# NumericalEarth/Breeze.jl

Measured on AMD Instinct MI355X. Metric: grid-cells advanced/sec (tendency+Poisson step), 512^3 anelastic, higher is better.
Workload: dtype f64

## Files before the change

### breeze.jl_amd/csrc/bz_tendency5_kernels.h

```cpp
#pragma once
#include "bz_internal.h"
#include "bz_weno.h"
#include "bz_tendency4_kernels.h"

#ifndef BZ_KO
#define BZ_KO 0
#endif
#ifndef BZ6_ROTATE_DUTY
#define BZ6_ROTATE_DUTY 0
#endif
#ifndef BZ6_UNROLL2
#define BZ6_UNROLL2 0
#endif
#ifndef BZ6_LDS_BARRIER
#define BZ6_LDS_BARRIER 0
#endif
__device__ __forceinline__ void bz6_barrier()
{
#if BZ6_LDS_BARRIER
    __builtin_amdgcn_fence(__ATOMIC_RELEASE, "workgroup", "local");
    __builtin_amdgcn_s_barrier();
    __builtin_amdgcn_fence(__ATOMIC_ACQUIRE, "workgroup", "local");
#else
    __syncthreads();
#endif
}
typedef long long ix_t;
typedef unsigned ix32_t;

struct LevRow5 {
    double rho, rrho;
    double rho_f, rrho_f;
    double Ax, Ay, Vinv_c;
    double pi;
    double Vinv_f, T_r;
    double pad[6];
};
struct Lev5 {
    const LevRow5 *p;
#ifdef __HIPCC__
    __device__ __forceinline__ double at(int k, int f) const { return ((ColPtr::cptr)(const double *)p)[(long long)k * 16 + f]; }
    __device__ __forceinline__ double rho(int k) const { return at(k, 0); }
    __device__ __forceinline__ double rrho(int k) const { return at(k, 1); }
    __device__ __forceinline__ double rho_f(int k) const { return at(k, 2); }
    __device__ __forceinline__ double rrho_f(int k) const { return at(k, 3); }
    __device__ __forceinline__ double Ax(int k) const { return at(k, 4); }
    __device__ __forceinline__ double Ay(int k) const { return at(k, 5); }
    __device__ __forceinline__ double Vinv_c(int k) const { return at(k, 6); }
    __device__ __forceinline__ double pi(int k) const { return at(k, 7); }
    __device__ __forceinline__ double Vinv_f(int k) const { return at(k, 8); }
    __device__ __forceinline__ double T_r(int k) const { return at(k, 9); }
#endif
};
static_assert(sizeof(LevRow5) == 16 * sizeof(double), "LevRow5 is sixteen reals");

#ifndef BZ_LEAN_WAVES
#define BZ_LEAN_WAVES (sizeof(double) == 8 ? 4 : 6)
#endif
#ifndef BZ5_ZERO_SHORTCUT
#define BZ5_ZERO_SHORTCUT 1
#endif
#ifndef BZ5_TOPS_AHEAD
#define BZ5_TOPS_AHEAD 1
#endif
#ifndef BZ6_W_WAVES
#define BZ6_W_WAVES 4
#endif
#ifndef BZ5_EB
#define BZ5_EB 64
#endif
#ifndef BZ5_RAW_LDS
#define BZ5_RAW_LDS 0
#endif
#ifndef BZ5_SCALAR_WAVES
#define BZ5_SCALAR_WAVES (sizeof(double) == 8 ? 4 : 6)
#endif

struct Lean5 {
    const double *ru, *rv, *rw;
    const double *pa, *pb;
    double *out;
    double *oa, *ob;
    double *T;
    ColPtr pi_dry;
    const LevRow5 *lev;
    int mforce;
    double cor_f;
    ColPtr Fu, Fv;
    ColPtr Su, Sv;
    const double *vel, *bT, *bq;
    const int *qstate;
    int xcd;
    int by0, bys;
};

__device__ __forceinline__ void bz_block5(const Lean5 &L, int &bx, int &by, int &bz)
{
    bx = blockIdx.x; by = blockIdx.y; bz = blockIdx.z;
    if (L.xcd) {
        const unsigned gx = gridDim.x, gy = gridDim.y;
        const unsigned W = gx * gy * gridDim.z;
        unsigned w = bx + gx * (by + gy * bz);
        w = (w & 7u) * (W >> 3) + (w >> 3);
        bx = (int)(w % gx);
        by = (int)((w / gx) % gy);
        bz = (int)(w / (gx * gy));
    }
    by = L.by0 + by * L.bys;
    bx = __builtin_amdgcn_readfirstlane(bx);
    by = __builtin_amdgcn_readfirstlane(by);
    bz = __builtin_amdgcn_readfirstlane(bz);
}

__device__ __forceinline__ void st_img5(double *__restrict__ f, long long n, double v, long long ox, long long oy)
{
    f[n] = v;
    if (ox) f[n + ox] = v;
    if (oy) {
        f[n + oy] = v;
        if (ox) f[n + ox + oy] = v;
    }
}


__device__ __forceinline__ double bz_temperature5(const DevGrid &g, double rth, double rq, int k, const ColPtr pi_dry)
{
    const double rho = g.rho[k], rrho = g.rrho[k];
    const double th = bz_cdiv(rth, rho, rrho), q = bz_cdiv(rq, rho, rrho);
    if (pi_dry.p && __all(q == 0.0)) return pi_dry[k] * th;
    const double qd = 1.0 - q;
    const double cpm = qd * g.cpd + q * g.cpv;
    return bz_exner_factor(g, k, q, cpm) * th;
}

__device__ __forceinline__ double bz_temperature5r(const DevGrid &g, double rth, double rq, int k, double rho, double rrho, double pi)
{
    const double th = bz_cdiv(rth, rho, rrho), q = bz_cdiv(rq, rho, rrho);
    if (__all(q == 0.0)) return pi * th;
    const double qd = 1.0 - q;
    const double cpm = qd * g.cpd + q * g.cpv;
    return bz_exner_factor(g, k, q, cpm) * th;
}

template <bool WY> __device__ __forceinline__ int by5_face(const DevGrid &g, int j) { return WY ? bz_buffer_face(j, g.Ny) : 3; }
template <bool WY> __device__ __forceinline__ int by5_center(const DevGrid &g, int j) { return WY ? bz_buffer_center(j, g.Ny) : 3; }
template <bool WY>
__device__ __forceinline__ double bz_up5y(double m3, double m2, double m1, double p0, double p1, double p2, bool left, int B)
{
    if constexpr (WY) return bz_upB(m3, m2, m1, p0, p1, p2, left, B);
    else return bz_up5(m3, m2, m1, p0, p1, p2, left);
}
template <bool WY>
__device__ __forceinline__ double bz_symm4y(double qm2, double qm1, double q0, double qp1, int B)
{
    if constexpr (WY) return (B == 3) ? bz_symm4(qm2, qm1, q0, qp1) : bz_symm2(qm1, q0);
    else return bz_symm4(qm2, qm1, q0, qp1);
}

template <int TY, bool WY, bool DRYQ>
__device__ __forceinline__ void k5_scalar_pair_body(const DevGrid &g, const Lean5 &F, int kchunk, const RKEpilogue &E, double *Tp, double *FYp, int *ZF, double *RAWp)
{
    constexpr bool Q = !DRYQ;
    constexpr int TR = TY + 6, TC = 72;
    constexpr int NHALO = TR * 70 - TY * 64;
    constexpr int NT = 64 * TY;
    constexpr int HPT = (NHALO + NT - 1) / NT;
    double(*T)[2][TR][TC] = (double(*)[2][TR][TC])Tp;
    double(*FY)[2][TY + 1][64] = (double(*)[2][TY + 1][64])FYp;
    double *__restrict__ RAW = RAWp;
    constexpr bool ZS = BZ5_ZERO_SHORTCUT && Q;

    int bx, by, bz;
    bz_block5(F, bx, by, bz);
    const int tx = threadIdx.x, ty = threadIdx.y, t = ty * 64 + tx;
    const int tyu = __builtin_amdgcn_readfirstlane(ty);
    const Lev5 LV{F.lev};
    const int i0 = bx * 64, j0 = by * TY;
    const int i = i0 + tx, j = j0 + ty;
    const int ic = min(i, g.Nx + 2), jc = min(j, g.Ny + 2);
    const int nact = min(64, g.Nx - i0);
    const int ie = i0 + nact, le = nact - 1;
    const int kbeg = bz * kchunk, kend = min(kbeg + kchunk, g.Nz);
    if (kbeg >= kend) return;
    const int Byj = by5_face<WY>(g, j0 + tyu), Byt = by5_face<WY>(g, j0 + TY);
    const unsigned sz = (unsigned)g.Sxy;
    const bool store = (i < g.Nx) && (j < g.Ny);
    const double *__restrict__ ru = F.ru, *__restrict__ rv = F.rv, *__restrict__ rw = F.rw;
    const double *__restrict__ pa = F.pa, *__restrict__ pb = F.pb;
    unsigned n = (unsigned)g.idx(ic, jc, kbeg);

    int hr[HPT], hc[HPT];
    unsigned hn[HPT];
    bool hok[HPT];
#pragma unroll
    for (int q = 0; q < HPT; ++q) {
        const int h = t + q * NT;
        hok[q] = h < NHALO;
        int r, c;
        if (h < 6 * 70) {
            const int rr = h / 70;
            c = h - rr * 70;
            r = (rr < 3) ? rr : TY + rr;
        } else {
            const int hh = h - 6 * 70;
            const int rr = hh / 6, cc = hh - rr * 6;
            r = 3 + rr;
            c = (cc < 3) ? cc : 64 + cc;
        }
        if (!hok[q]) { r = 0; c = 0; }
        hr[q] = r; hc[q] = c;
        const int gi = min(i0 - 3 + c, g.Nx + 2), gj = min(j0 - 3 + r, g.Ny + 2);
        hn[q] = (unsigned)g.idx(gi, gj, kbeg);
    }
    const unsigned ntop0 = (unsigned)g.idx(ic, min(j0 + TY, g.Ny), kbeg);

    double a[6], b[6];
    double araw[3] = {0.0, 0.0, 0.0};
#pragma unroll
    for (int s = 0; s < 6; ++s) {
        const double rh = g.rho[kbeg + s - 3], rr = g.rrho[kbeg + s - 3];
        const double raw = pa[n + s * sz - 3 * sz];
        a[s] = bz_cdiv(raw, rh, rr);
        if (DRYQ && s >= 3) araw[s - 3] = raw;
        if constexpr (Q) {
            const double rawb = pb[n + s * sz - 3 * sz];
            b[s] = bz_cdiv(rawb, rh, rr);
            if (BZ5_RAW_LDS && s >= 3) { RAW[((s - 3) * 2 + 0) * NT + t] = raw; RAW[((s - 3) * 2 + 1) * NT + t] = rawb; }
        } else b[s] = 0.0;
    }
    double fza, fzb = 0.0;
    {
        const double wt = bz_cdiv(rw[n], g.rho_f[kbeg], g.rrho_f[kbeg]);
        const bool left = wt > 0.0;
        const int B = bz_buffer_face(kbeg, g.Nz);
        const double cf = g.Az * wt, rf = g.rho_f[kbeg];
        fza = rf * (cf * bz_upB(a[0], a[1], a[2], a[3], a[4], a[5], left, B));
        if constexpr (Q) fzb = rf * (cf * bz_upB(b[0], b[1], b[2], b[3], b[4], b[5], left, B));
    }
    int zrun = 0;
    if constexpr (ZS) {
#pragma unroll
        for (int s = 0; s < 6; ++s) zrun = (b[s] == 0.0) ? zrun + 1 : 0;
        if (t < 3) ZF[t] = 1;
        __syncthreads();
    }
    T[0][0][ty + 3][tx + 3] = a[3];
    if constexpr (Q) T[0][1][ty + 3][tx + 3] = b[3];
    {
        const double rh = g.rho[kbeg], rr = g.rrho[kbeg];
        bool z0 = (b[3] == 0.0);
#pragma unroll
        for (int q = 0; q < HPT; ++q)
            if (hok[q]) {
                T[0][0][hr[q]][hc[q]] = bz_cdiv(pa[hn[q]], rh, rr);
                if constexpr (Q) {
                    const double hbv = bz_cdiv(pb[hn[q]], rh, rr);
                    T[0][1][hr[q]][hc[q]] = hbv;
                    z0 = z0 && (hbv == 0.0);
                }
            }
        if (ZS && !__all(z0) && tx == 0) ZF[0] = 0;
    }
    __syncthreads();

    double ea = 0.0, eb = 0.0;
    int buf = 0;
    double ru_n = ru[n], rv_n = rv[n], rw_n = rw[n + sz];
    double rvtop_n = (tyu == 0 || (Q && tyu == TY / 2)) ? rv[ntop0] : 0.0;
    double ta_nx = 0.0, tb_nx = 0.0;
    if constexpr (BZ5_TOPS_AHEAD) { ta_nx = pa[n + 3 * sz]; if constexpr (Q) tb_nx = pb[n + 3 * sz]; }
    for (int k = kbeg; k < kend; ++k, n += sz) {
        double ha[HPT], hb[HPT];
        const unsigned lev = (unsigned)(k + 1 - kbeg) * sz;
        double ta_raw, tb_raw = 0.0;
        if constexpr (BZ5_TOPS_AHEAD) {
            ta_raw = ta_nx; tb_raw = tb_nx;
            const unsigned up = (k + 4 <= g.Nz + g.Hz - 1) ? 4 * sz : 3 * sz;
            ta_nx = pa[n + up];
            if constexpr (Q) tb_nx = pb[n + up];
        } else { ta_raw = pa[n + 3 * sz]; if constexpr (Q) tb_raw = pb[n + 3 * sz]; }
        const int lv3 = (ZS || (Q && BZ5_RAW_LDS)) ? (k - kbeg) % 3 : 0;
        bool zxy = false;
        if constexpr (ZS) {
            if (t == 0) ZF[(lv3 + 2) % 3] = 1;
            zxy = __builtin_amdgcn_readfirstlane(ZF[lv3]) != 0;
        }
#pragma unroll
        for (int q = 0; q < HPT; ++q) {
            if (BZ_KO & 2) { ha[q] = ta_raw; hb[q] = tb_raw; }
            else { ha[q] = hok[q] ? pa[hn[q] + lev] : 0.0; hb[q] = (Q && hok[q]) ? pb[hn[q] + lev] : 0.0; }
        }
        const double u0a = (BZ_KO & 16) ? ta_raw : (E.mode == 2) ? E.u0[n] : 0.0, u0b = (BZ_KO & 16) ? tb_raw : (Q && E.mode == 2) ? E.u0b[n] : 0.0;
        const double ru_t = ru_n, rv_t = rv_n, rw_t = rw_n, rvtop = rvtop_n;
        const int turn = (k - kbeg) & (TY - 1);
        const bool duty_a = tyu == turn, duty_b = Q && tyu == ((turn + TY / 2) & (TY - 1));
        if (BZ_KO & 32) { ru_n = ta_raw * 1e-3; rv_n = tb_raw; rw_n = ta_raw * 1e-4; } else {
        ru_n = ru[n + sz]; rv_n = rv[n + sz]; rw_n = rw[n + 2 * sz]; }
        {
            const int turn_n = (turn + 1) & (TY - 1);
            const bool duty_n = tyu == turn_n || (Q && tyu == ((turn_n + TY / 2) & (TY - 1)));
            rvtop_n = duty_n ? rv[ntop0 + lev] : 0.0;
        }
        const double rho = LV.rho(k), rrho = LV.rrho(k), Ax_k = LV.Ax(k), Ay_k = LV.Ay(k), Vi_k = LV.Vinv_c(k);
        const double rho1 = LV.rho(k + 1), rrho1 = LV.rrho(k + 1), rhof1 = LV.rho_f(k + 1), rrhof1 = LV.rrho_f(k + 1);
        const double rho3 = LV.rho(k + 3), rrho3 = LV.rrho(k + 3);
        if (((k - kbeg) & (BZ5_EB - 1)) == 0) {
            const int kk = min(k + (tx & (BZ5_EB - 1)), kend - 1);
            const long long ne = g.idx(ie, jc, kk);
            const double rhk = g.rho[kk], rrk = g.rrho[kk];
            const double ue = bz_cdiv(ru[ne], rhk, rrk);
            const bool le_ = ue > 0.0;
            const double cf = g.Ax[kk] * ue;
            ea = rhk * (cf * bz_up5(bz_cdiv(pa[ne - 3], rhk, rrk), bz_cdiv(pa[ne - 2], rhk, rrk), bz_cdiv(pa[ne - 1], rhk, rrk),
                                    bz_cdiv(pa[ne], rhk, rrk), bz_cdiv(pa[ne + 1], rhk, rrk), bz_cdiv(pa[ne + 2], rhk, rrk), le_));
            if constexpr (Q)
            eb = rhk * (cf * bz_up5(bz_cdiv(pb[ne - 3], rhk, rrk), bz_cdiv(pb[ne - 2], rhk, rrk), bz_cdiv(pb[ne - 1], rhk, rrk),
                                    bz_cdiv(pb[ne], rhk, rrk), bz_cdiv(pb[ne + 1], rhk, rrk), bz_cdiv(pb[ne + 2], rhk, rrk), le_));
        }
        const int src = (k - kbeg) & (BZ5_EB - 1);
        const double ut = bz_cdiv(ru_t, rho, rrho), vt = bz_cdiv(rv_t, rho, rrho);
        const double wt = bz_cdiv(rw_t, rhof1, rrhof1);
        const double cfx = Ax_k * ut, cfy = Ay_k * vt, cfz = g.Az * wt, rf = rhof1;
        const bool lx = ut > 0.0, ly = vt > 0.0, lz = wt > 0.0;
        const int Bz = bz_buffer_face(k + 1, g.Nz);
        double cfy2 = 0.0;
        bool ly2 = false;
        if (duty_a || duty_b) {
            const double vtop = bz_cdiv(rvtop, rho, rrho);
            ly2 = vtop > 0.0;
            cfy2 = Ay_k * vtop;
        }
        const int c = tx + 3;
        double fxa, fya, fza_hi, fxb, fyb, fzb_hi;
        const double ta = bz_cdiv(ta_raw, rho3, rrho3);
        {
            const double(*Tk)[TC] = T[buf][0];
            const double *rr_ = Tk[ty + 3] + tx;
            fxa = rho * (cfx * bz_up5(rr_[0], rr_[1], rr_[2], a[3], rr_[4], rr_[5], lx));
            fya = rho * (cfy * bz_up5y<WY>(Tk[ty][c], Tk[ty + 1][c], Tk[ty + 2][c], a[3], Tk[ty + 4][c], Tk[ty + 5][c], ly, Byj));
            FY[buf][0][ty][tx] = fya;
            if (duty_a)
                FY[buf][0][TY][tx] = rho * (cfy2 * bz_up5y<WY>(Tk[TY][c], Tk[TY + 1][c], Tk[TY + 2][c], Tk[TY + 3][c], Tk[TY + 4][c], Tk[TY + 5][c], ly2, Byt));
            fza_hi = rf * (cfz * bz_upB(a[1], a[2], a[3], a[4], a[5], ta, lz, Bz));
        }
        double tb = 0.0;
        fxb = 0.0; fyb = 0.0; fzb_hi = 0.0;
        if constexpr (Q) {
        tb = bz_cdiv(tb_raw, rho3, rrho3);
        bool zz = false;
        if constexpr (ZS) {
            zrun = (tb == 0.0) ? min(zrun + 1, 6) : 0;
            zz = __all(zrun >= 6);
        }
        if (zxy) {
            fxb = 0.0; fyb = 0.0;
            FY[buf][1][ty][tx] = 0.0;
            if (duty_b) FY[buf][1][TY][tx] = 0.0;
        } else {
            const double(*Tk)[TC] = T[buf][1];
            const double *rr_ = Tk[ty + 3] + tx;
            if (BZ_KO & 128) { fxb = rho * (cfx * b[3]); fyb = rho * (cfy * b[3]); } else {
            fxb = rho * (cfx * bz_up5(rr_[0], rr_[1], rr_[2], b[3], rr_[4], rr_[5], lx));
            fyb = rho * (cfy * bz_up5y<WY>(Tk[ty][c], Tk[ty + 1][c], Tk[ty + 2][c], b[3], Tk[ty + 4][c], Tk[ty + 5][c], ly, Byj)); }
            FY[buf][1][ty][tx] = fyb;
            if (duty_b)
                FY[buf][1][TY][tx] = rho * (cfy2 * bz_up5y<WY>(Tk[TY][c], Tk[TY + 1][c], Tk[TY + 2][c], Tk[TY + 3][c], Tk[TY + 4][c], Tk[TY + 5][c], ly2, Byt));
        }
        if (zz) fzb_hi = 0.0;
        else fzb_hi = (BZ_KO & 128) ? rf * (cfz * b[3]) : rf * (cfz * bz_upB(b[1], b[2], b[3], b[4], b[5], tb, lz, Bz));
        }
        double pa_n, pb_n;
        if constexpr (DRYQ) { pa_n = araw[0]; pb_n = b[3]; araw[0] = araw[1]; araw[1] = araw[2]; araw[2] = ta_raw; }
        else if (BZ_KO & 4) { pa_n = a[3]; pb_n = b[3]; }
        else if constexpr (BZ5_RAW_LDS) {
            double *ra = RAW + (lv3 * 2 + 0) * NT + t, *rb = ra + NT;
            pa_n = *ra; pb_n = *rb;
            *ra = ta_raw; *rb = tb_raw;
        } else { pa_n = pa[n]; pb_n = pb[n]; }
        T[buf ^ 1][0][ty + 3][tx + 3] = a[4];
        if constexpr (Q) T[buf ^ 1][1][ty + 3][tx + 3] = b[4];
        {
            const double rh = rho1, rr = rrho1;
            bool z1 = (b[4] == 0.0);
#pragma unroll
            for (int q = 0; q < HPT; ++q)
                if (hok[q]) {
                    T[buf ^ 1][0][hr[q]][hc[q]] = bz_cdiv(ha[q], rh, rr);
                    if constexpr (Q) {
                        const double hbv = bz_cdiv(hb[q], rh, rr);
                        T[buf ^ 1][1][hr[q]][hc[q]] = hbv;
                        z1 = z1 && (hbv == 0.0);
                    }
                }
            if (ZS && !__all(z1) && tx == 0) ZF[(lv3 + 1) % 3] = 0;
        }
        if (!(BZ_KO & 64)) __syncthreads();
        {
            double na = __shfl_down(fxa, 1);
            const double xa = __shfl(ea, src);
            if (tx == le) na = xa;
            const double dya = FY[buf][0][ty + 1][tx] - fya;
            const double Vi = Vi_k;
            const double ga = -(Vi * ((na - fxa) + dya + (fza_hi - fza)));
            double gb = 0.0;
            if constexpr (Q) {
                double nb = __shfl_down(fxb, 1);
                const double xb = __shfl(eb, src);
                if (tx == le) nb = xb;
                const double dyb = FY[buf][1][ty + 1][tx] - fyb;
                gb = -(Vi * ((nb - fxb) + dyb + (fzb_hi - fzb)));
            }
            if (store) {
                const double rth = bz_rk_apply_pre(E.mode, E.dt, E.alpha, E.oma, u0a, E.u0_out, ga, pa_n, n);
                F.oa[n] = rth;
                if constexpr (Q) {
                    const double rq = bz_rk_apply_pre(E.mode, E.dt, E.alpha, E.oma, u0b, E.u0b_out, gb, pb_n, n);
                    F.ob[n] = rq;
                }
            }
        }
        fza = fza_hi; fzb = fzb_hi;
#pragma unroll
        for (int s = 0; s < 5; ++s) { a[s] = a[s + 1]; b[s] = b[s + 1]; }
        a[5] = ta; b[5] = tb;
        buf ^= 1;
    }
}


template <bool DRYQ, bool GUARD>
__device__ __forceinline__ bool bz_lean_skip(const Lean5 &F)
{
    if constexpr (!GUARD) return false;
    const bool dry = F.qstate != nullptr && __builtin_amdgcn_readfirstlane(*F.qstate) == 1;
    return dry != DRYQ;
}
template <int TY, bool WY = false, bool DRYQ = false, bool GUARD = true>
__global__ __launch_bounds__(64 * TY) __attribute__((amdgpu_waves_per_eu(BZ5_SCALAR_WAVES, BZ5_SCALAR_WAVES))) void k5_scalar_pair(DevGrid g, Lean5 F, int kchunk, RKEpilogue E)
{
    constexpr int TR = TY + 6, TC = 72;
    __shared__ double T[2 * 2 * TR * TC];
    __shared__ double FY[2 * 2 * (TY + 1) * 64];
    __shared__ int ZF[3];
    __shared__ double RAW[(!DRYQ && BZ5_RAW_LDS) ? 3 * 2 * 64 * TY : 1];
    if (bz_lean_skip<DRYQ, GUARD>(F)) return;
    k5_scalar_pair_body<TY, WY, DRYQ>(g, F, kchunk, E, T, FY, ZF, RAW);
}

template <int KIND>
__device__ __forceinline__ double flux_x_lean(const DevGrid &g, const Tend3Fields &F, const double *__restrict__ m, int i, int j, int k, int By = 3)
{
    const long long n = g.idx(i, j, k);
    const double a = (KIND == T3_V && By != 3) ? bz_symm2(g.Ax[k] * F.ru[n - g.Sx], g.Ax[k] * F.ru[n]) : adv_x<KIND>(g, F, n, k);
    const double rh = (KIND == T3_W) ? g.rho_f[k] : g.rho[k], rr = (KIND == T3_W) ? g.rrho_f[k] : g.rrho[k];
    if constexpr (KIND == T3_U)
        return a * bz_up5(bz_cdiv(m[n - 2], rh, rr), bz_cdiv(m[n - 1], rh, rr), bz_cdiv(m[n], rh, rr), bz_cdiv(m[n + 1], rh, rr),
                          bz_cdiv(m[n + 2], rh, rr), bz_cdiv(m[n + 3], rh, rr), a > 0.0);
    else
        return a * bz_up5(bz_cdiv(m[n - 3], rh, rr), bz_cdiv(m[n - 2], rh, rr), bz_cdiv(m[n - 1], rh, rr), bz_cdiv(m[n], rh, rr),
                          bz_cdiv(m[n + 1], rh, rr), bz_cdiv(m[n + 2], rh, rr), a > 0.0);
}


template <int TY, bool MF = false, bool WY = false, bool ST = false>
__global__ __launch_bounds__(64 * TY, BZ_LEAN_WAVES) void k6_u(DevGrid g, Lean5 L, int kchunk, RKEpilogue E)
{
    static_assert(!(ST && WY), "stored-velocity instantiations: periodic / slab rows");
    constexpr int TR = TY + 6, TC = 72, NT = 64 * TY;
    constexpr int NH1 = TR * 70 - TY * 64;
    constexpr int NH2 = 3 * (TY + 1) + 64 + 3 * TY;
    static_assert(NH1 <= NT && NH2 <= NT, "one frame cell of each kind per thread");
    __shared__ double U[2][TR][TC];
    __shared__ double RU[2][TY][TC];
    __shared__ double RV[2][TY + 1][TC];
    __shared__ double RW[2][TY][TC];
    __shared__ double FY[2][TY + 1][64];
    int bx, by, bz;
    bz_block5(L, bx, by, bz);
    const int tx = threadIdx.x, ty = threadIdx.y, t = ty * 64 + tx, tc = tx + 3;
    const int i0 = bx * 64, j0 = by * TY;
    const int i = i0 + tx, j = j0 + ty;
    const int ic = min(i, g.Nx + 2), jc = min(j, g.Ny + 2);
    const int ie = i0 - 1, le = 0;
    const int kbeg = bz * kchunk, kend = min(kbeg + kchunk, g.Nz);
    if (kbeg >= kend) return;
    const ix_t sz = (ix_t)g.Sxy;
    const bool store = (i < g.Nx) && (j < g.Ny);
    const double *__restrict__ ru = L.ru, *__restrict__ rv = L.rv, *__restrict__ rw = L.rw;
    const double *__restrict__ vel = ST ? L.vel : L.ru;
    Tend3Fields F;
    F.ru = L.ru; F.rv = L.rv; F.rw = L.rw; F.u = F.v = F.w = F.T = F.q = nullptr; F.c = ST ? L.vel : nullptr; F.G = L.out;
    ix_t n = (ix_t)g.idx(ic, jc, kbeg);
    const bool h1ok = !(BZ_KO & 32768) && t < NH1;
    int h1r = 0, h1c = 0;
    {
        const int h = h1ok ? t : 0;
        if (h < 6 * 70) { const int rr = h / 70; h1c = h - rr * 70; h1r = (rr < 3) ? rr : TY + rr; }
        else { const int hh = h - 6 * 70, rr = hh / 6, cc = hh - rr * 6; h1r = 3 + rr; h1c = (cc < 3) ? cc : 64 + cc; }
    }
    const ix_t h1n = (ix_t)g.idx(min(i0 - 3 + h1c, g.Nx + 2), min(j0 - 3 + h1r, g.Ny + 2), kbeg);
    const bool h1raw = h1ok && h1r >= 3 && h1r < TY + 3 && (h1c == 2 || h1c == 67 || h1c == 68);
    const bool h2ok = !(BZ_KO & 32768) && t < NH2;
    int h2sel = 0, h2r = 0, h2c = 0;
    {
        const int id = h2ok ? t : 0;
        if (id < 3 * (TY + 1)) { h2r = id / 3; const int cc = id - 3 * h2r; h2c = (cc < 2) ? 1 + cc : 67; }
        else if (id < 3 * (TY + 1) + 64) { h2r = TY; h2c = 3 + (id - 3 * (TY + 1)); }
        else { h2sel = 1; const int m = id - 3 * (TY + 1) - 64; h2r = m / 3; const int cc = m - 3 * h2r; h2c = (cc < 2) ? 1 + cc : 67; }
    }
    const double *__restrict__ h2src = h2sel ? rw : rv;
    const ix_t h2n = (ix_t)g.idx(min(i0 - 3 + h2c, g.Nx + 2), min(j0 + h2r, g.Ny + 2), kbeg) + (h2sel ? sz : (ix_t)0);

    double r[6];
#pragma unroll
    for (int s = 0; s < 6; ++s) r[s] = ST ? vel[n + s * sz - 3 * sz] : bz_cdiv(ru[n + s * sz - 3 * sz], g.rho[kbeg + s - 3], g.rrho[kbeg + s - 3]);
    double fz_lo = vflux<T3_U>(g, F, n, kbeg, r[0], r[1], r[2], r[3], r[4], r[5]);
    double q0 = ru[n], q1 = ru[n + sz], q2 = ru[n + 2 * sz];
    U[0][ty + 3][tc] = r[3];
    RU[0][ty][tc] = q0;
    RV[0][ty][tc] = rv[n];
    RW[0][ty][tc] = rw[n + sz];
    if (h1ok) {
        const double raw = (ST && !h1raw) ? 0.0 : ru[h1n];
        U[0][h1r][h1c] = ST ? vel[h1n] : bz_cdiv(raw, g.rho[kbeg], g.rrho[kbeg]);
        if (h1raw) RU[0][h1r - 3][h1c] = raw;
    }
    if (h2ok) { if (h2sel) RW[0][h2r][h2c] = h2src[h2n]; else RV[0][h2r][h2c] = h2src[h2n]; }
    double tcur_raw = ru[n + 3 * sz];
    double tcur_v = ST ? vel[n + 3 * sz] : 0.0;
    double u0cur = (E.mode == 2) ? E.u0[n] : 0.0;
    __syncthreads();

    double edge = 0.0;
    int buf = 0;
#if BZ6_UNROLL2
#pragma unroll 2
#endif
    for (int k = kbeg; k < kend; ++k, n += sz) {
        const ix_t lev1 = (ix_t)(k + 1 - kbeg) * sz;
        const double p_top = ST ? ru[n + sz] : ru[n + ((k + 4 <= g.Nz + g.Hz - 1) ? 4 * sz : 3 * sz)];
        const double p_topv = ST ? vel[n + ((k + 4 <= g.Nz + g.Hz - 1) ? 4 * sz : 3 * sz)] : 0.0;
        const double p_h1 = (BZ_KO & 256) ? p_top : h1ok ? (ST ? vel : ru)[h1n + lev1] : 0.0;
        const double p_h1raw = (ST && h1raw) ? ru[h1n + lev1] : 0.0;
        const double p_h2 = (BZ_KO & 512) ? p_top : h2ok ? h2src[h2n + lev1] : 0.0;
        const double p_rv = (BZ_KO & 1024) ? p_top * 0.5 : rv[n + sz], p_rw = (BZ_KO & 1024) ? p_top * 0.25 : rw[n + 2 * sz];
        const double p_u0 = (BZ_KO & 2048) ? p_top : (E.mode == 2) ? E.u0[n + sz] : 0.0;
        if (((k - kbeg) & (BZ5_EB - 1)) == 0) {
            const int kk = min(k + (tx & (BZ5_EB - 1)), kend - 1);
            edge = ST ? flux_x_at<T3_U>(g, F, ie, jc, kk) : flux_x_lean<T3_U>(g, F, ru, ie, jc, kk);
        }
        const int src = (k - kbeg) & (BZ5_EB - 1);
        const double Ax = g.Ax[k], Ay = g.Ay[k], Az = g.Az;
        const double c0 = r[3];
        const double(*Uk)[TC] = U[buf];
        const double *rur = RU[buf][ty] + tc, *ur = Uk[ty + 3] + tc;
        const double ax = bz_symm4(Ax * rur[-1], Ax * q0, Ax * rur[1], Ax * rur[2]);
        const double fx = ax * bz_up5(ur[-2], ur[-1], c0, ur[1], ur[2], ur[3], ax > 0.0);
        const double *rvr = RV[buf][ty] + tc;
        const double ay = bz_symm4(Ay * rvr[-2], Ay * rvr[-1], Ay * rvr[0], Ay * rvr[1]);
        const double fy = ay * bz_up5y<WY>(Uk[ty][tc], Uk[ty + 1][tc], Uk[ty + 2][tc], c0, Uk[ty + 4][tc], Uk[ty + 5][tc], ay > 0.0, by5_face<WY>(g, __builtin_amdgcn_readfirstlane(j)));
        FY[buf][ty][tx] = fy;
        if (ty == (BZ6_ROTATE_DUTY ? ((k - kbeg) & (TY - 1)) : 0) && !(BZ_KO & 4096)) {
            const double *rvt = RV[buf][TY] + tc;
            const double at = bz_symm4(Ay * rvt[-2], Ay * rvt[-1], Ay * rvt[0], Ay * rvt[1]);
            FY[buf][TY][tx] = at * bz_up5y<WY>(Uk[TY][tc], Uk[TY + 1][tc], Uk[TY + 2][tc], Uk[TY + 3][tc], Uk[TY + 4][tc], Uk[TY + 5][tc], at > 0.0,
                                               by5_face<WY>(g, j0 + TY));
        }
        const double tnew = ST ? tcur_v : bz_cdiv(tcur_raw, g.rho[k + 3], g.rrho[k + 3]);
        const double *rwr = RW[buf][ty] + tc;
        const double wt = bz_symm4(Az * rwr[-2], Az * rwr[-1], Az * rwr[0], Az * rwr[1]);
        const double fz_hi = wt * bz_upB(r[1], r[2], r[3], r[4], r[5], tnew, wt > 0.0, bz_buffer_face(k + 1, g.Nz));
        U[buf ^ 1][ty + 3][tc] = r[4];
        RU[buf ^ 1][ty][tc] = ST ? p_top : q1;
        RV[buf ^ 1][ty][tc] = p_rv;
        RW[buf ^ 1][ty][tc] = p_rw;
        if (h1ok) {
            U[buf ^ 1][h1r][h1c] = ST ? p_h1 : bz_cdiv(p_h1, g.rho[k + 1], g.rrho[k + 1]);
            if (h1raw) RU[buf ^ 1][h1r - 3][h1c] = ST ? p_h1raw : p_h1;
        }
        if (h2ok) { if (h2sel) RW[buf ^ 1][h2r][h2c] = p_h2; else RV[buf ^ 1][h2r][h2c] = p_h2; }
        if (!(BZ_KO & 16384) && (!(BZ_KO & 8192) || ((k - kbeg) & 1))) bz6_barrier();
        {
            double nb = __shfl_up(fx, 1);
            const double e = __shfl(edge, src);
            if (tx == le) nb = e;
            const double dx = fx - nb;
            const double dy = (BZ_KO & 16384) ? 0.5 * fy : FY[buf][ty + 1][tx] - fy;
            double Gu = -(g.Vinv_c[k] * (dx + dy + (fz_hi - fz_lo)));
            if constexpr (MF) {
                if (L.mforce & 1) {
                    const double *rv0 = RV[buf][ty] + tc, *rv1 = RV[buf][ty + 1] + tc;
                    const double a = (rv0[-1] + rv1[-1]) / 2, b = (rv0[0] + rv1[0]) / 2;
                    Gu -= -L.cor_f * ((a + b) / 2);
                }
                if (L.mforce & (2 | 8)) {
                    const double rho = g.rho[k];
                    double tot = (L.mforce & 8) ? rho * L.Su[k] : 0.0;
                    if (L.mforce & 2) tot = (L.mforce & 8) ? tot + rho * L.Fu[k] : rho * L.Fu[k];
                    Gu += tot;
                }
            }
            if (store) L.out[n] = (ST && E.mode == 0) ? Gu : bz_rk_apply_pre(E.mode, E.dt, E.alpha, E.oma, u0cur, E.u0_out, Gu, q0, n);
        }
        fz_lo = fz_hi;
#pragma unroll
        for (int s = 0; s < 5; ++s) r[s] = r[s + 1];
        r[5] = tnew;
        if (ST) q0 = p_top;
        else { q0 = q1; q1 = q2; q2 = tcur_raw; tcur_raw = p_top; }
        u0cur = p_u0;
        if (ST) tcur_v = p_topv;
        buf ^= 1;
    }
}


template <int TY, bool MF = false, bool WY = false, bool ST = false>
__global__ __launch_bounds__(64 * TY, ((MF && WY) ? 4 : BZ_LEAN_WAVES)) void k6_v(DevGrid g, Lean5 L, int kchunk, RKEpilogue E)
{
    static_assert(!(ST && WY), "stored-velocity instantiations: periodic / slab rows");
    constexpr int RV = TY + 6, RM = TY + 4;
    constexpr int TC = 72;
    __shared__ double Tv[2][RV][TC];
    __shared__ double Tm[2][3][RM][64];
    __shared__ double FY[2][TY + 1][64];
    constexpr int NT = 64 * TY, NFR = 16 * 64, HPT = (NFR + NT - 1) / NT;
    int bx, by, bz;
    bz_block5(L, bx, by, bz);
    const int tx = threadIdx.x, ty = threadIdx.y, t = ty * 64 + tx, tc = tx + 3;
    const int i0 = bx * 64, j0 = by * TY;
    const int i = i0 + tx, j = j0 + ty;
    const int ic = min(i, g.Nx + 2), jc = min(j, g.Ny + 2);
    const int nact = min(64, g.Nx - i0);
    const int ie = i0 + nact, le = nact - 1;
    const int kbeg = bz * kchunk, kend = min(kbeg + kchunk, g.Nz);
    if (kbeg >= kend) return;
    const ix_t sz = (ix_t)g.Sxy;
    const bool store = (i < g.Nx) && (j < g.Ny) && !(WY && j == 0);
    const int ju = __builtin_amdgcn_readfirstlane(j);
    const int Bf = by5_face<WY>(g, ju), Bc = by5_center<WY>(g, ju), Bc0 = by5_center<WY>(g, j0 - 1);
    const double *__restrict__ ru = L.ru, *__restrict__ rv = L.rv, *__restrict__ rw = L.rw;
    const double *__restrict__ vel = ST ? L.vel : L.rv;
    Tend3Fields F;
    F.ru = L.ru; F.rv = L.rv; F.rw = L.rw; F.u = F.v = F.w = F.T = F.q = nullptr; F.c = ST ? L.vel : nullptr; F.G = L.out;
    const double Az = g.Az;
    ix_t n = (ix_t)g.idx(ic, jc, kbeg);

    bool hok[HPT];
    int hsel[HPT], hrow[HPT];
    ix_t hn[HPT];
    const double *hsrc[HPT];
#pragma unroll
    for (int q = 0; q < HPT; ++q) {
        const int h = t + q * NT;
        hok[q] = h < NFR;
        const int id = __builtin_amdgcn_readfirstlane(hok[q] ? (h >> 6) : 0);
        int sel, row, grow;
        if (id < 6) { sel = 0; row = (id < 3) ? id : TY + id; grow = j0 - 3 + row; }
        else if (id < 9) { sel = 1; const int m = id - 6; row = (m < 2) ? m : TY + 2; grow = j0 - 2 + row; }
        else if (id < 13) { sel = 2; const int m = id - 9; row = (m < 2) ? m : TY + m; grow = j0 - 2 + row; }
        else { sel = 3; const int m = id - 13; row = (m < 2) ? m : TY + 2; grow = j0 - 2 + row; }
        hsel[q] = sel; hrow[q] = row;
        hsrc[q] = (sel == 1) ? ru : (sel == 3) ? rw : (ST && sel == 0) ? vel : rv;
        hn[q] = (ix_t)g.idx(min(i0 + tx, g.Nx + 2), min(grow, g.Ny + 2), kbeg) + (sel == 3 ? sz : (ix_t)0);
    }
    auto frame_load = [&](int q, ix_t lev) -> double { return hsrc[q][hn[q] + lev]; };
    auto frame_store = [&](int b, int q, double raw, int klev) {
        if (hsel[q] == 0) Tv[b][hrow[q]][tc] = ST ? raw : bz_cdiv(raw, g.rho[klev], g.rrho[klev]);
        else Tm[b][hsel[q] - 1][hrow[q]][tx] = ((hsel[q] == 1) ? g.Ax[klev] : (hsel[q] == 2) ? g.Ay[klev] : Az) * raw;
    };

    const bool sok = t < 5 * TY;
    const int srow = sok ? t / 5 : 0, scc = sok ? t % 5 : 0, scol = (scc < 3) ? scc : 64 + scc;
    const ix_t sn = (ix_t)g.idx(min(i0 - 3 + scol, g.Nx + 2), min(j0 + srow, g.Ny + 2), kbeg);

    double r[6];
#pragma unroll
    for (int s = 0; s < 6; ++s) r[s] = ST ? vel[n + s * sz - 3 * sz] : bz_cdiv(rv[n + s * sz - 3 * sz], g.rho[kbeg + s - 3], g.rrho[kbeg + s - 3]);
    double fz_lo;
    if (WY && Bf != 3) {
        const double wt0 = bz_symm2(Az * rw[n - (ix_t)g.Sx], Az * rw[n]);
        fz_lo = wt0 * bz_upB(r[0], r[1], r[2], r[3], r[4], r[5], wt0 > 0.0, bz_buffer_face(kbeg, g.Nz));
    } else fz_lo = vflux<T3_V>(g, F, n, kbeg, r[0], r[1], r[2], r[3], r[4], r[5]);
    double q0 = rv[n], q1 = rv[n + sz], q2 = rv[n + 2 * sz];
    Tv[0][ty + 3][tc] = r[3];
    if (sok) Tv[0][srow + 3][scol] = ST ? vel[sn] : bz_cdiv(rv[sn], g.rho[kbeg], g.rrho[kbeg]);
    Tm[0][0][ty + 2][tx] = g.Ax[kbeg] * ru[n];
    Tm[0][1][ty + 2][tx] = g.Ay[kbeg] * q0;
    Tm[0][2][ty + 2][tx] = Az * rw[n + sz];
#pragma unroll
    for (int q = 0; q < HPT; ++q)
        if (hok[q]) frame_store(0, q, frame_load(q, 0), kbeg);
    __syncthreads();

    double tcur_raw = rv[n + 3 * sz];
    double tcur_v = ST ? vel[n + 3 * sz] : 0.0;
    double u0cur = (E.mode == 2) ? E.u0[n] : 0.0;
    double edge = 0.0;
    int buf = 0;
    for (int k = kbeg; k < kend; ++k, n += sz) {
        const ix_t lev = (ix_t)(k + 1 - kbeg) * sz;
        double hnext[HPT];
#pragma unroll
        for (int q = 0; q < HPT; ++q) hnext[q] = hok[q] ? frame_load(q, lev) : 0.0;
        const double p_side = sok ? (ST ? vel : rv)[sn + lev] : 0.0;
        const double p_top = ST ? rv[n + sz] : rv[n + ((k + 4 <= g.Nz + g.Hz - 1) ? 4 * sz : 3 * sz)];
        const double p_topv = ST ? vel[n + ((k + 4 <= g.Nz + g.Hz - 1) ? 4 * sz : 3 * sz)] : 0.0;
        const double p_u0 = (E.mode == 2) ? E.u0[n + sz] : 0.0;
        const double tnew_raw = tcur_raw, u0v = u0cur;
        const double ru_n = g.Ax[k + 1] * ru[n + sz], rw_n = Az * rw[n + 2 * sz];
        double cor_u = 0.0, cg1 = 0.0, cg3 = 0.0;
        if constexpr (MF) { if ((L.mforce & 1) && tx == 63) { const ix_t sy = (ix_t)g.Sx; cg1 = ru[n - sy + 1]; cg3 = ru[n + 1]; } }
        if (((k - kbeg) & (BZ5_EB - 1)) == 0) {
            const int kk = min(k + (tx & (BZ5_EB - 1)), kend - 1);
            edge = ST ? flux_x_at<T3_V>(g, F, ie, jc, kk) : flux_x_lean<T3_V>(g, F, rv, ie, jc, kk, Bf);
        }
        const int src = (k - kbeg) & (BZ5_EB - 1);
        const double rho = g.rho[k];
        const double c0 = r[3];
        const double(*V)[TC] = Tv[buf];
        const double *vrow = V[ty + 3] + tc;
        const double(*MU)[64] = Tm[buf][0];
        const double(*MV)[64] = Tm[buf][1];
        const double(*MW)[64] = Tm[buf][2];
        const double ut = bz_symm4y<WY>(MU[ty][tx], MU[ty + 1][tx], MU[ty + 2][tx], MU[ty + 3][tx], Bf);
        const double fx = ut * bz_up5(vrow[-3], vrow[-2], vrow[-1], c0, vrow[1], vrow[2], ut > 0.0);
        const double vt = (!WY || Bc == 3) ? bz_symm4(MV[ty + 1][tx], MV[ty + 2][tx], MV[ty + 3][tx], MV[ty + 4][tx]) : bz_symm2(MV[ty + 2][tx], MV[ty + 3][tx]);
        const double fy = vt * bz_up5y<WY>(V[ty + 1][tc], V[ty + 2][tc], c0, V[ty + 4][tc], V[ty + 5][tc], V[ty + 6][tc], vt > 0.0, Bc);
        FY[buf][ty + 1][tx] = fy;
        if (ty == 0 && !(BZ_KO & 4096)) {
            const double vb = (!WY || Bc0 == 3) ? bz_symm4(MV[0][tx], MV[1][tx], MV[2][tx], MV[3][tx]) : bz_symm2(MV[1][tx], MV[2][tx]);
            FY[buf][0][tx] = vb * bz_up5y<WY>(V[0][tc], V[1][tc], V[2][tc], V[3][tc], V[4][tc], V[5][tc], vb > 0.0, Bc0);
        }
        const double tnew = ST ? tcur_v : bz_cdiv(tnew_raw, g.rho[k + 3], g.rrho[k + 3]);
        const double wt = bz_symm4y<WY>(MW[ty][tx], MW[ty + 1][tx], MW[ty + 2][tx], MW[ty + 3][tx], Bf);
        const double fz_hi = wt * bz_upB(r[1], r[2], r[3], r[4], r[5], tnew, wt > 0.0, bz_buffer_face(k + 1, g.Nz));
        if constexpr (MF) {
            if (L.mforce & 1) {
                const double Axk = g.Ax[k];
                const double l1 = MU[ty + 1][tx + 1], l3 = MU[ty + 2][tx + 1];
                const double c1 = (tx == 63) ? Axk * cg1 : l1, c3 = (tx == 63) ? Axk * cg3 : l3;
                cor_u = (((MU[ty + 1][tx] + c1) / 2 + (MU[ty + 2][tx] + c3) / 2) / 2) / Axk;
            }
        }
        Tv[buf ^ 1][ty + 3][tc] = r[4];
        if (sok) Tv[buf ^ 1][srow + 3][scol] = ST ? p_side : bz_cdiv(p_side, g.rho[k + 1], g.rrho[k + 1]);
        Tm[buf ^ 1][0][ty + 2][tx] = ru_n;
        Tm[buf ^ 1][1][ty + 2][tx] = g.Ay[k + 1] * (ST ? p_top : q1);
        Tm[buf ^ 1][2][ty + 2][tx] = rw_n;
#pragma unroll
        for (int q = 0; q < HPT; ++q)
            if (hok[q]) frame_store(buf ^ 1, q, hnext[q], k + 1);
        bz6_barrier();
        {
            double nb = __shfl_down(fx, 1);
            const double e = __shfl(edge, src);
            if (tx == le) nb = e;
            const double dx = nb - fx;
            const double dy = fy - FY[buf][ty][tx];
            double Gv = -(g.Vinv_c[k] * (dx + dy + (fz_hi - fz_lo)));
            if constexpr (MF) {
                if (L.mforce & 1) Gv -= L.cor_f * cor_u;
                if (L.mforce & (4 | 16)) {
                    double tot = (L.mforce & 16) ? rho * L.Sv[k] : 0.0;
                    if (L.mforce & 4) tot = (L.mforce & 16) ? tot + rho * L.Fv[k] : rho * L.Fv[k];
                    Gv += tot;
                }
            }
            if (store) L.out[n] = (ST && E.mode == 0) ? Gv : bz_rk_apply_pre(E.mode, E.dt, E.alpha, E.oma, u0v, E.u0_out, Gv, q0, n);
            if constexpr (WY) {
                if (i < g.Nx && j == 0) L.out[n] = 0.0;
                if (i < g.Nx && j == g.Ny - 1) L.out[n + (ix_t)g.Sx] = 0.0;
            }
        }
        fz_lo = fz_hi;
        if (ST) q0 = p_top;
        else { q0 = q1; q1 = q2; q2 = tnew_raw; tcur_raw = p_top; }
        u0cur = p_u0;
        if (ST) tcur_v = p_topv;
#pragma unroll
        for (int s = 0; s < 5; ++s) r[s] = r[s + 1];
        r[5] = tnew;
        buf ^= 1;
    }
}

__device__ __forceinline__ double buoyancy5(const DevGrid &g, double rth, double rq, int k, double rho, double rrho, double pi, double T_ref)
{
    const double th = bz_cdiv(rth, rho, rrho), q = bz_cdiv(rq, rho, rrho);
    double T;
    if (__all(q == 0.0)) T = pi * th;
    else {
        const double qd = 1.0 - q;
        const double cpm = qd * g.cpd + q * g.cpv;
        T = bz_exner_factor(g, k, q, cpm) * th;
    }
    const double Rm = (1.0 - q) * g.Rd + q * g.Rv;
    const double rhop = rho * (g.Rd * T_ref / (Rm * T) - 1.0);
    return -g.g * rhop;
}


template <int TY, bool WY = false, bool DRYQ = false, bool GUARD = true, int BM = 4>
__global__ __launch_bounds__(64 * TY, BZ6_W_WAVES) void k6_w(DevGrid g, Lean5 L, int kchunk, RKEpilogue E)
{
    constexpr bool ST = BM != 4;
    static_assert(!(ST && (WY || DRYQ || GUARD)), "stored-velocity instantiations: periodic / slab rows, no moisture-scan dispatch");
    if (bz_lean_skip<DRYQ, GUARD>(L)) return;
    constexpr int TR = TY + 6, TC = 72, NT = 64 * TY, NH = TR * 70 - TY * 64;
    static_assert(NH <= NT, "one frame cell per thread");
    __shared__ double T[2][TR][TC];
    __shared__ double FY[2][TY + 1][64];
    int bx, by, bz;
    bz_block5(L, bx, by, bz);
    const int tx = threadIdx.x, ty = threadIdx.y, t = ty * 64 + tx, tc = tx + 3;
    const int i0 = bx * 64, j0 = by * TY;
    const int i = i0 + tx, j = j0 + ty;
    const int ic = min(i, g.Nx + 2), jc = min(j, g.Ny + 2);
    const int nact = min(64, g.Nx - i0);
    const int ie = i0 + nact, le = nact - 1;
    const int kbeg = 1 + bz * kchunk, kend = min(kbeg + kchunk, g.Nz);
    if (kbeg >= kend) return;
    const ix32_t sz = (ix32_t)g.Sxy;
    const bool store = (i < g.Nx) && (j < g.Ny);
    const double *__restrict__ ru = L.ru, *__restrict__ rv = L.rv, *__restrict__ rw = L.rw;
    const double *__restrict__ pa = L.pa, *__restrict__ pb = L.pb;
    const double *__restrict__ vel = ST ? L.vel : L.rw;
    const double *__restrict__ bT = L.bT, *__restrict__ bq = L.bq;
    const Lev5 LV{L.lev};
    constexpr bool dryq = DRYQ;
    Tend3Fields F;
    F.ru = L.ru; F.rv = L.rv; F.rw = L.rw; F.u = F.v = F.w = F.T = F.q = nullptr; F.c = ST ? L.vel : nullptr; F.G = L.out;
    const double Az = g.Az;
    ix32_t n = (ix32_t)g.idx(ic, jc, kbeg);
    const bool hok = t < NH;
    int hr = 0, hc = 0;
    {
        const int h = hok ? t : 0;
        if (h < 6 * 70) { const int rr = h / 70; hc = h - rr * 70; hr = (rr < 3) ? rr : TY + rr; }
        else { const int hh = h - 6 * 70, rr = hh / 6, cc = hh - rr * 6; hr = 3 + rr; hc = (cc < 3) ? cc : 64 + cc; }
    }
    const ix32_t hn = (ix32_t)g.idx(min(i0 - 3 + hc, g.Nx + 2), min(j0 - 3 + hr, g.Ny + 2), kbeg);
    const ix32_t ntop0 = (ix32_t)g.idx(ic, min(j0 + TY, g.Ny), kbeg);
    const bool top = (ty == 0);

    double wr[6], qu[4], qv[4], qt[4], qw[4];
    double raw0 = 0.0, raw1 = 0.0, raw2 = 0.0;
#pragma unroll
    for (int s = 0; s < 6; ++s) {
        const double x = rw[n + s * sz - 3 * sz];
        wr[s] = ST ? vel[n + s * sz - 3 * sz] : bz_cdiv(x, LV.rho_f(kbeg + s - 3), LV.rrho_f(kbeg + s - 3));
        if (s >= 1 && s <= 4) qw[s - 1] = Az * x;
        if (s == 3) raw0 = x;
        if (s == 4) raw1 = x;
        if (s == 5) raw2 = x;
    }
#pragma unroll
    for (int s = 0; s < 4; ++s) {
        const int kk = kbeg - 2 + s;
        const double Axk = ST ? g.Ax[kk] : LV.Ax(kk), Ayk = ST ? g.Ay[kk] : LV.Ay(kk);
        qu[s] = Axk * ru[n + s * sz - 2 * sz];
        qv[s] = Ayk * rv[n + s * sz - 2 * sz];
        qt[s] = top ? Ayk * rv[ntop0 + s * sz - 2 * sz] : 0.0;
    }
    double fz_lo, b_lo, r_lo = 0.0;
    {
        const int B = bz_buffer_center(kbeg - 1, g.Nz);
        const double wt = (B == 3) ? bz_symm4(qw[0], qw[1], qw[2], qw[3]) : bz_symm2(qw[1], qw[2]);
        fz_lo = wt * bz_upB(wr[0], wr[1], wr[2], wr[3], wr[4], wr[5], wt > 0.0, B);
        if constexpr (BM == 4) b_lo = buoyancy5(g, pa[n - sz], dryq ? 0.0 : pb[n - sz], kbeg - 1, LV.rho(kbeg - 1), LV.rrho(kbeg - 1), LV.pi(kbeg - 1), LV.T_r(kbeg - 1));
        else if constexpr (BM == 0) b_lo = buoyancy3(g, bT[n - sz], bq[n - sz], kbeg - 1);
        else if constexpr (BM == 3) b_lo = bz_buoyancy(g, bT, bq, (long long)(n - sz), kbeg - 1);
        else if constexpr (BM == 2) { b_lo = bT[n - sz] - g.p_r[kbeg - 1]; r_lo = bq[n - sz] - g.rho[kbeg - 1]; }
        else b_lo = 0.0;
    }
    T[0][ty + 3][tc] = wr[3];
    if (hok) T[0][hr][hc] = ST ? vel[hn] : bz_cdiv(rw[hn], LV.rho_f(kbeg), LV.rrho_f(kbeg));
    double tcur_raw = rw[n + 3 * sz];
    double tcur_v = ST ? vel[n + 3 * sz] : 0.0;
    double u0cur = (E.mode == 2) ? E.u0[n] : 0.0;
    __syncthreads();

    double edge = 0.0;
    int buf = 0;
    for (int k = kbeg; k < kend; ++k, n += sz) {
        const ix32_t lev = (ix32_t)(k - kbeg) * sz;
        const double p_h = hok ? (ST ? vel : rw)[hn + lev + sz] : 0.0;
        const double p_top = rw[n + ((k + 4 <= g.Nz + g.Hz) ? 4 * sz : 3 * sz)];
        const double p_topv = ST ? vel[n + ((k + 4 <= g.Nz + g.Hz) ? 4 * sz : 3 * sz)] : 0.0;
        const double Tcur = (BM == 1) ? 0.0 : (ST ? bT : pa)[n], rqcur = (BM == 1) ? 0.0 : ST ? bq[n] : dryq ? 0.0 : pb[n];
        const double p_u0 = (E.mode == 2) ? E.u0[n + sz] : 0.0;
        const double Axn = ST ? g.Ax[k + 2] : LV.Ax(k + 2), Ayn = ST ? g.Ay[k + 2] : LV.Ay(k + 2);
        const double qun = Axn * ru[n + 2 * sz], qvn = Ayn * rv[n + 2 * sz];
        const double qtn = top ? Ayn * rv[ntop0 + lev + 2 * sz] : 0.0;
        if (((k - kbeg) & (BZ5_EB - 1)) == 0) {
            const int kk = min(k + (tx & (BZ5_EB - 1)), kend - 1);
            edge = ST ? flux_x_at<T3_W>(g, F, ie, jc, kk) : flux_x_lean<T3_W>(g, F, rw, ie, jc, kk);
        }
        const int src = (k - kbeg) & (BZ5_EB - 1);
        const int Bf = bz_buffer_face(k, g.Nz);
        const double w0 = wr[3];
        const double qwnew = Az * (ST ? rw[n + 2 * sz] : raw2);
        const double uold = ST ? rw[n] : raw0;
        const double(*Tk)[TC] = T[buf];
        const double *wrow = Tk[ty + 3] + tc;
        const double ut = (Bf == 3) ? bz_symm4(qu[0], qu[1], qu[2], qu[3]) : bz_symm2(qu[1], qu[2]);
        const double fx = ut * bz_up5(wrow[-3], wrow[-2], wrow[-1], w0, wrow[1], wrow[2], ut > 0.0);
        const double vt = (Bf == 3) ? bz_symm4(qv[0], qv[1], qv[2], qv[3]) : bz_symm2(qv[1], qv[2]);
        const double fy = vt * bz_up5y<WY>(Tk[ty][tc], Tk[ty + 1][tc], Tk[ty + 2][tc], w0, Tk[ty + 4][tc], Tk[ty + 5][tc], vt > 0.0, by5_face<WY>(g, __builtin_amdgcn_readfirstlane(j)));
        FY[buf][ty][tx] = fy;
        if (top && !(BZ_KO & 4096)) {
            const double v2 = (Bf == 3) ? bz_symm4(qt[0], qt[1], qt[2], qt[3]) : bz_symm2(qt[1], qt[2]);
            FY[buf][TY][tx] = v2 * bz_up5y<WY>(Tk[TY][tc], Tk[TY + 1][tc], Tk[TY + 2][tc], Tk[TY + 3][tc], Tk[TY + 4][tc], Tk[TY + 5][tc], v2 > 0.0,
                                               by5_face<WY>(g, j0 + TY));
        }
        const double wnew = ST ? tcur_v : bz_cdiv(tcur_raw, LV.rho_f(k + 3), LV.rrho_f(k + 3));
        double fz_hi;
        {
            const int B = bz_buffer_center(k, g.Nz);
            const double wt = (B == 3) ? bz_symm4(qw[1], qw[2], qw[3], qwnew) : bz_symm2(qw[2], qw[3]);
            fz_hi = wt * bz_upB(wr[1], wr[2], wr[3], wr[4], wr[5], wnew, wt > 0.0, B);
        }
        double b_hi = 0.0, r_hi = 0.0;
        if constexpr (BM == 4) b_hi = buoyancy5(g, Tcur, rqcur, k, LV.rho(k), LV.rrho(k), LV.pi(k), LV.T_r(k));
        else if constexpr (BM == 0) b_hi = buoyancy3(g, Tcur, rqcur, k);
        else if constexpr (BM == 3) b_hi = bz_buoyancy(g, bT, bq, (long long)n, k);
        else if constexpr (BM == 2) { b_hi = Tcur - g.p_r[k]; r_hi = rqcur - g.rho[k]; }
        T[buf ^ 1][ty + 3][tc] = wr[4];
        if (hok) T[buf ^ 1][hr][hc] = ST ? p_h : bz_cdiv(p_h, LV.rho_f(k + 1), LV.rrho_f(k + 1));
        bz6_barrier();
        {
            double nb = __shfl_down(fx, 1);
            const double e = __shfl(edge, src);
            if (tx == le) nb = e;
            const double dx = nb - fx;
            const double dy = FY[buf][ty + 1][tx] - fy;
            const double adv = -((ST ? g.Vinv_f[k] : LV.Vinv_f(k)) * (dx + dy + (fz_hi - fz_lo)));
            double Gval;
            if constexpr (BM == 2) Gval = adv - (b_hi - b_lo) * g.rdzf[k] - g.g * ((r_hi + r_lo) / 2.0);
            else if constexpr (BM == 1) Gval = adv;
            else Gval = adv + 0.5 * (b_lo + b_hi);
            if (store)
                L.out[n] = (ST && E.mode == 0) ? Gval : bz_rk_apply_pre(E.mode, E.dt, E.alpha, E.oma, u0cur, E.u0_out, Gval, uold, n);
        }
        fz_lo = fz_hi;
        b_lo = b_hi;
        r_lo = r_hi;
#pragma unroll
        for (int s = 0; s < 3; ++s) { qu[s] = qu[s + 1]; qv[s] = qv[s + 1]; qt[s] = qt[s + 1]; qw[s] = qw[s + 1]; }
        qu[3] = qun; qv[3] = qvn; qt[3] = qtn; qw[3] = qwnew;
        raw0 = raw1; raw1 = raw2; raw2 = tcur_raw;
        tcur_raw = p_top; u0cur = p_u0;
        if (ST) tcur_v = p_topv;
#pragma unroll
        for (int s = 0; s < 5; ++s) wr[s] = wr[s + 1];
        wr[5] = wnew;
        buf ^= 1;
    }
}
```

Baseline: 4.189 billion.

## Re-read kernel args from kernarg segment to cut SGPR/VGPR pressure in k6_w

Kernel arguments used inside the vertical loop (edge flux fields, RK epilogue parameters, output pointer, grid constants) are now re-read from the kernarg segment, with empty asm barriers so the compiler cannot keep them live across the loop. The aim is to lower register pressure and improve occupancy or avoid spills. Face-velocity sums for the vertical flux are rebuilt from raw values with pinned FMAs, and the products for the next level are deferred until after the barrier, moving multiplies to a point where fewer values are live. The scalar reloads cost a little extra, and the changed FMA grouping can alter floating-point rounding.

```diff
diff --git a/breeze.jl_amd/csrc/bz_tendency5_kernels.h b/breeze.jl_amd/csrc/bz_tendency5_kernels.h
--- a/breeze.jl_amd/csrc/bz_tendency5_kernels.h
+++ b/breeze.jl_amd/csrc/bz_tendency5_kernels.h
@@ -111,6 +111,35 @@
     by = __builtin_amdgcn_readfirstlane(by);
     bz = __builtin_amdgcn_readfirstlane(bz);
 }
+
+struct K6Args { DevGrid g; Lean5 L; int kchunk; RKEpilogue E; };
+#ifdef __HIPCC__
+__device__ __forceinline__ const K6Args &bz_args_here()
+{
+    auto p = __builtin_amdgcn_kernarg_segment_ptr();
+    asm volatile("" : "+s"(p));
+    return *(const K6Args *)p;
+}
+#endif
+
+#ifdef __HIPCC__
+__device__ __forceinline__ double bz_mad_pinned(double a, double b, double c)
+{
+#ifdef BZ_NO_CONTRACT
+    return a * b + c;
+#else
+    return fma(a, b, c);
+#endif
+}
+__device__ __forceinline__ double bz_symm4_sums(double inner, double outer)
+{
+#ifdef BZ_CENTERED2
+    return 0.5 * inner;
+#else
+    return (7.0 / 12.0) * inner - (1.0 / 12.0) * outer;
+#endif
+}
+#endif
 
 __device__ __forceinline__ void st_img5(double *__restrict__ f, long long n, double v, long long ox, long long oy)
 {
@@ -792,10 +821,10 @@
     if (__all(q == 0.0)) T = pi * th;
     else {
         const double qd = 1.0 - q;
-        const double cpm = qd * g.cpd + q * g.cpv;
+        const double cpm = bz_mad_pinned(q, g.cpv, qd * g.cpd);
         T = bz_exner_factor(g, k, q, cpm) * th;
     }
-    const double Rm = (1.0 - q) * g.Rd + q * g.Rv;
+    const double Rm = bz_mad_pinned(q, g.Rv, (1.0 - q) * g.Rd);
     const double rhop = rho * (g.Rd * T_ref / (Rm * T) - 1.0);
     return -g.g * rhop;
 }
@@ -829,8 +858,6 @@
     const double *__restrict__ bT = L.bT, *__restrict__ bq = L.bq;
     const Lev5 LV{L.lev};
     constexpr bool dryq = DRYQ;
-    Tend3Fields F;
-    F.ru = L.ru; F.rv = L.rv; F.rw = L.rw; F.u = F.v = F.w = F.T = F.q = nullptr; F.c = ST ? L.vel : nullptr; F.G = L.out;
     const double Az = g.Az;
     ix32_t n = (ix32_t)g.idx(ic, jc, kbeg);
     const bool hok = t < NH;
@@ -846,11 +873,14 @@
 
     double wr[6], qu[4], qv[4], qt[4], qw[4];
     double raw0 = 0.0, raw1 = 0.0, raw2 = 0.0;
+    double rawm2 = 0.0, rawm1 = 0.0;
 #pragma unroll
     for (int s = 0; s < 6; ++s) {
         const double x = rw[n + s * sz - 3 * sz];
         wr[s] = ST ? vel[n + s * sz - 3 * sz] : bz_cdiv(x, LV.rho_f(kbeg + s - 3), LV.rrho_f(kbeg + s - 3));
         if (s >= 1 && s <= 4) qw[s - 1] = Az * x;
+        if (s == 1) rawm2 = x;
+        if (s == 2) rawm1 = x;
         if (s == 3) raw0 = x;
         if (s == 4) raw1 = x;
         if (s == 5) raw2 = x;
@@ -866,7 +896,8 @@
     double fz_lo, b_lo, r_lo = 0.0;
     {
         const int B = bz_buffer_center(kbeg - 1, g.Nz);
-        const double wt = (B == 3) ? bz_symm4(qw[0], qw[1], qw[2], qw[3]) : bz_symm2(qw[1], qw[2]);
+        const double inner = bz_mad_pinned(Az, rawm1, qw[2]);
+        const double wt = (B == 3) ? bz_symm4_sums(inner, bz_mad_pinned(Az, rawm2, qw[3])) : 0.5 * inner;
         fz_lo = wt * bz_upB(wr[0], wr[1], wr[2], wr[3], wr[4], wr[5], wt > 0.0, B);
         if constexpr (BM == 4) b_lo = buoyancy5(g, pa[n - sz], dryq ? 0.0 : pb[n - sz], kbeg - 1, LV.rho(kbeg - 1), LV.rrho(kbeg - 1), LV.pi(kbeg - 1), LV.T_r(kbeg - 1));
         else if constexpr (BM == 0) b_lo = buoyancy3(g, bT[n - sz], bq[n - sz], kbeg - 1);
@@ -885,22 +916,28 @@
     int buf = 0;
     for (int k = kbeg; k < kend; ++k, n += sz) {
         const ix32_t lev = (ix32_t)(k - kbeg) * sz;
+        auto u0p = (const __attribute__((address_space(1))) double *)bz_args_here().E.u0;
         const double p_h = hok ? (ST ? vel : rw)[hn + lev + sz] : 0.0;
         const double p_top = rw[n + ((k + 4 <= g.Nz + g.Hz) ? 4 * sz : 3 * sz)];
         const double p_topv = ST ? vel[n + ((k + 4 <= g.Nz + g.Hz) ? 4 * sz : 3 * sz)] : 0.0;
         const double Tcur = (BM == 1) ? 0.0 : (ST ? bT : pa)[n], rqcur = (BM == 1) ? 0.0 : ST ? bq[n] : dryq ? 0.0 : pb[n];
-        const double p_u0 = (E.mode == 2) ? E.u0[n + sz] : 0.0;
         const double Axn = ST ? g.Ax[k + 2] : LV.Ax(k + 2), Ayn = ST ? g.Ay[k + 2] : LV.Ay(k + 2);
-        const double qun = Axn * ru[n + 2 * sz], qvn = Ayn * rv[n + 2 * sz];
-        const double qtn = top ? Ayn * rv[ntop0 + lev + 2 * sz] : 0.0;
+        const double run = ru[n + 2 * sz], rvn = rv[n + 2 * sz];
+        const double rvtn = top ? rv[ntop0 + lev + 2 * sz] : 0.0;
+        asm volatile("" : "+s"(u0p));
+        const double p_u0 = (E.mode == 2) ? u0p[n + sz] : 0.0;
         if (((k - kbeg) & (BZ5_EB - 1)) == 0) {
             const int kk = min(k + (tx & (BZ5_EB - 1)), kend - 1);
-            edge = ST ? flux_x_at<T3_W>(g, F, ie, jc, kk) : flux_x_lean<T3_W>(g, F, rw, ie, jc, kk);
+            const K6Args &A = bz_args_here();
+            Tend3Fields F;
+            F.ru = A.L.ru; F.rv = A.L.rv; F.rw = A.L.rw; F.u = F.v = F.w = F.T = F.q = nullptr; F.c = ST ? A.L.vel : nullptr; F.G = A.L.out;
+            edge = ST ? flux_x_at<T3_W>(A.g, F, ie, jc, kk) : flux_x_lean<T3_W>(A.g, F, A.L.rw, ie, jc, kk);
         }
         const int src = (k - kbeg) & (BZ5_EB - 1);
         const int Bf = bz_buffer_face(k, g.Nz);
         const double w0 = wr[3];
-        const double qwnew = Az * (ST ? rw[n + 2 * sz] : raw2);
+        const double rawk2 = ST ? rw[n + 2 * sz] : raw2;
+        const double qwnew = Az * rawk2;
         const double uold = ST ? rw[n] : raw0;
         const double(*Tk)[TC] = T[buf];
         const double *wrow = Tk[ty + 3] + tc;
@@ -914,34 +951,43 @@
             FY[buf][TY][tx] = v2 * bz_up5y<WY>(Tk[TY][tc], Tk[TY + 1][tc], Tk[TY + 2][tc], Tk[TY + 3][tc], Tk[TY + 4][tc], Tk[TY + 5][tc], v2 > 0.0,
                                                by5_face<WY>(g, j0 + TY));
         }
+        const K6Args &A = bz_args_here();
         const double wnew = ST ? tcur_v : bz_cdiv(tcur_raw, LV.rho_f(k + 3), LV.rrho_f(k + 3));
         double fz_hi;
         {
             const int B = bz_buffer_center(k, g.Nz);
-            const double wt = (B == 3) ? bz_symm4(qw[1], qw[2], qw[3], qwnew) : bz_symm2(qw[2], qw[3]);
+            const double inner = qw[2] + qw[3];
+            const double wt = (B == 3) ? bz_symm4_sums(inner, bz_mad_pinned(Az, rawk2, qw[1])) : 0.5 * inner;
             fz_hi = wt * bz_upB(wr[1], wr[2], wr[3], wr[4], wr[5], wnew, wt > 0.0, B);
         }
         double b_hi = 0.0, r_hi = 0.0;
-        if constexpr (BM == 4) b_hi = buoyancy5(g, Tcur, rqcur, k, LV.rho(k), LV.rrho(k), LV.pi(k), LV.T_r(k));
+        if constexpr (BM == 4) b_hi = buoyancy5(A.g, Tcur, rqcur, k, LV.rho(k), LV.rrho(k), LV.pi(k), LV.T_r(k));
         else if constexpr (BM == 0) b_hi = buoyancy3(g, Tcur, rqcur, k);
         else if constexpr (BM == 3) b_hi = bz_buoyancy(g, bT, bq, (long long)n, k);
-        else if constexpr (BM == 2) { b_hi = Tcur - g.p_r[k]; r_hi = rqcur - g.rho[k]; }
+        else if constexpr (BM == 2) { b_hi = Tcur - A.g.p_r[k]; r_hi = rqcur - A.g.rho[k]; }
         T[buf ^ 1][ty + 3][tc] = wr[4];
         if (hok) T[buf ^ 1][hr][hc] = ST ? p_h : bz_cdiv(p_h, LV.rho_f(k + 1), LV.rrho_f(k + 1));
+        auto outp = (__attribute__((address_space(1))) double *)A.L.out;
+        int emode = A.E.mode;
+        double edt = A.E.dt, ealpha = A.E.alpha, eoma = A.E.oma, Vinv = ST ? A.g.Vinv_f[k] : LV.Vinv_f(k);
+        asm volatile("" : "+s"(outp), "+s"(emode), "+s"(edt), "+s"(ealpha), "+s"(eoma), "+s"(Vinv));
         bz6_barrier();
+        double qun, qvn, qtn;
         {
             double nb = __shfl_down(fx, 1);
             const double e = __shfl(edge, src);
             if (tx == le) nb = e;
             const double dx = nb - fx;
             const double dy = FY[buf][ty + 1][tx] - fy;
-            const double adv = -((ST ? g.Vinv_f[k] : LV.Vinv_f(k)) * (dx + dy + (fz_hi - fz_lo)));
+            qun = Axn * run; qvn = Ayn * rvn; qtn = Ayn * rvtn;
+            asm volatile("" : "+v"(qun), "+v"(qvn), "+v"(qtn));
+            const double adv = -(Vinv * (dx + dy + (fz_hi - fz_lo)));
             double Gval;
-            if constexpr (BM == 2) Gval = adv - (b_hi - b_lo) * g.rdzf[k] - g.g * ((r_hi + r_lo) / 2.0);
+            if constexpr (BM == 2) Gval = adv - (b_hi - b_lo) * A.g.rdzf[k] - A.g.g * ((r_hi + r_lo) / 2.0);
             else if constexpr (BM == 1) Gval = adv;
             else Gval = adv + 0.5 * (b_lo + b_hi);
             if (store)
-                L.out[n] = (ST && E.mode == 0) ? Gval : bz_rk_apply_pre(E.mode, E.dt, E.alpha, E.oma, u0cur, E.u0_out, Gval, uold, n);
+                outp[n] = (ST && emode == 0) ? Gval : bz_rk_apply_pre(emode, edt, ealpha, eoma, u0cur, A.E.u0_out, Gval, uold, n);
         }
         fz_lo = fz_hi;
         b_lo = b_hi;
```

New measurement: 4.199 billion (median of 6 runs). No clear change (+0.2%).
